# szbonaldo/FedMLP

Hardware: AMD Instinct MI355X
Metric: images/sec/client (ICH 224x224 bs=128) at 1/2/4/8 GPUs; mAP vs ref (higher is better)
Workload: dtype f32; 1 GPU; FedMLP stage1 step, Resnet18, ICH-shaped synthetic 3x224x224, C=5, bs=128, one client per GPU, FedAvg all-reduce every 40 steps + once at end; parallelism=clients1, rccl_ranks=1, stream_mode=default: frozen teacher + weight gradients on the engine's side stream, arithmetic=fp32 operands+sums; products as 6 exact bf16 partials on the bf16 matrix pipe

## Files before the change

### fedmlp_amd/_lib.py

```python
import ctypes as C
import os

_HERE = os.path.dirname(os.path.abspath(__file__))
LIB_PATH = os.environ.get("FEDMLP_HIP_LIB") or os.path.join(_HERE, "libfedmlp_hip.so")

FM_MAX_CLASSES = 32
FM_MAX_GROUPS = 8
FM_COMM_ID_BYTES = 128


class FmConfig(C.Structure):
    _fields_ = [("model", C.c_int32), ("n_classes", C.c_int32), ("in_h", C.c_int32),
                ("in_w", C.c_int32), ("max_images", C.c_int32), ("reserved", C.c_int32 * 3),
                ("stream", C.c_void_p)]


class FmAdam(C.Structure):
    _fields_ = [("lr", C.c_float), ("beta1", C.c_float), ("beta2", C.c_float),
                ("eps", C.c_float), ("weight_decay", C.c_float)]


class FmSgd(C.Structure):
    _fields_ = [("lr", C.c_float), ("momentum", C.c_float), ("dampening", C.c_float),
                ("weight_decay", C.c_float), ("nesterov", C.c_int32)]
# ... 86 lines not shown
    "fm_comm_preflight": (C.c_int, []),
    "fm_comm_unique_id": (C.c_int, [C.POINTER(C.c_uint8)]),
    "fm_comm_init": (C.c_int, [_P, C.POINTER(C.c_uint8), _I32, _I32]),
    "fm_comm_destroy": (C.c_int, [_P]),
    "fm_comm_size": (C.c_int, [_P]),
    "fm_fedavg_allreduce": (C.c_int, [_P, C.c_float]),
    "fm_fedavg_tao": (C.c_int, [_P, C.POINTER(C.c_double), C.c_double, _F, C.POINTER(C.c_double)]),
    "fm_fedavg_proto": (C.c_int, [_P, _P, C.c_double, _F, _P]),
    "fm_profile_ops": (C.c_int, [_P, _I32, C.c_char_p, _I32]),
    "fm_debug_num_convs": (C.c_int, [_P]),
    "fm_debug_conv_info": (C.c_int, [_P, _I32, C.POINTER(_I32)]),
    "fm_debug_conv": (C.c_int, [_P, _I32, _I32, _P, _P, _P, _I32, _I32, _P]),
    "fm_debug_conv_fwd": (C.c_int, [_P, _I32, _P, _P, _I32, _I32, _P, _P, _P, _I32, _P, _P, _P, _P]),
    "fm_debug_block_dgrad": (C.c_int, [_P, _I32, _P, _P, _P, _I32]),
    "fm_debug_conv_planes": (C.c_int, [_P, _I32, _P, _I32, _P, _P, _P, _P, _I32, _P, _P]),
    "fm_debug_conv_arm": (C.c_int, [_P, _I32, _I32, _I32]),
    "fm_debug_pw": (C.c_int, [_P, _I32, _I32, _P, _P, _P, _I32, _I32, _P, _P, _P, _P]),
    "fm_debug_pw_fwd": (C.c_int, [_P, _I32, _P, _P, _I32, _I32, _P, _P, _P, _I32, _P, _P, _P, _P]),
    "fm_debug_proj_bwd": (C.c_int, [_P, _I32, _I32, _P, _P, _P, _P, _P, _I32, _I32, _P, _P]),
    "fm_debug_exp_bwd": (C.c_int, [_P, _I32, _P, _P, _P, _P, _P, _I32, _I32, _P, _P]),
    "fm_debug_get_grads": (C.c_int, [_P, _P]),
    "fm_debug_optim_arena": (C.c_int, [_P, _I32, C.POINTER(_P), C.POINTER(_I64)]),
    "fm_debug_entry_spans": (C.c_int, [_P, _P, _I32]),
    "fm_debug_activation": (C.c_int, [_P, _I32, _I32, _I32, _P, C.POINTER(_I32)]),
    "fm_debug_stem_masks": (C.c_int, [_P, _I32, _I32, _P, _P]),
    "fm_debug_lose_part": (C.c_int, [_I32]),
    "fm_debug_lane_delay": (C.c_int, [_P, _I32, _I64, _I32]),
    "fm_debug_lane_points": (C.c_int, [_P, C.POINTER(_I64), _I32]),
    "fm_debug_drop_wait": (C.c_int, [_P, _I32, _I32]),
    "fm_debug_ew": (C.c_int, [_P, _I32, C.POINTER(_P), C.POINTER(_I32), _F]),
# ... 59 lines not shown
```

### fedmlp_amd/csrc/common.h

```cpp
#pragma once
#include <hip/hip_runtime.h>
#include <stdint.h>

#include <stdlib.h>

typedef float f32x4 __attribute__((ext_vector_type(4)));

#ifndef FM_F32_FAST_SWISH
#define FM_F32_FAST_SWISH 1
#endif
#ifdef __HIPCC__
__device__ __forceinline__ float fm_swish_f32(float v)
{
#if FM_F32_FAST_SWISH
    return v * __builtin_amdgcn_rcpf(1.f + __expf(-v));
#else
    return v / (1.f + expf(-v));
#endif
}
#endif


#ifndef FM_MFMA_SPLIT_DEFAULT
#define FM_MFMA_SPLIT_DEFAULT 6
// ... 151 lines not shown
    int Ho, Wo, Hi, Wi, Ci, stride, pad, ksz;
    long long npix, xpix;
    int pix_per_split;
    int tilesM, tilesN, nblk_n;
    int sp;
    int nimg, Qtot, q_per_split, splits, xcd_remap;
    unsigned magW, magH;
};
struct StemRowsParams {
    const unsigned short* Xp;
    const unsigned short* Wst;
    float* Y;
    const float* scale;
    const float* shift;
    float* stats;
    int imgs, imgs_per_group, Hp, Wp, Ho, Wo, relu, sp;
    long long plane_bytes;
};
bool stem_rows_takes(int k, int stride, int cout, int hout, int wout, long long plane_bytes);
int stem_rows_stats_tiles(int imgs_per_group, int hout);
void launch_stem_rows(StemRowsParams p, hipStream_t s);
void k_stem_weight_planes(const float* w, unsigned short* dst, int Kw, hipStream_t s);
int launch_pwgrad(PwgradParams p, size_t slab_floats, hipStream_t s);
bool pwgrad_ring_takes(const PwgradParams& p);
int launch_pwgrad_ring(PwgradParams p, size_t slab_floats, hipStream_t s);
bool pwgrad_takes(int M, int Ci, int ksz, long long npix, long long xpix, int Wi, int pad);
void launch_igemm(IgemmParams p, int groups, hipStream_t s);
void launch_pconv(IgemmParams p, int groups, hipStream_t s);
bool pconv_takes(int M, int Ci, long long xp_pix, int Wi);
bool pconv_uses_ts(const IgemmParams& p);
// ... 20 lines not shown
```

### fedmlp_amd/csrc/engine.hip

```cpp
#include <math.h>
#include <stdio.h>
#include <string.h>

#include <algorithm>
#include <string>
#include <unordered_map>
#include <vector>

#include "../../include/fedmlp_hip.h"
#include "../../include/fedmlp_hip_debug.h"
#include "../../include/fedmlp_hip_rofl.h"
#include "../../include/fedmlp_hip_drift.h"
#include "comm.h"
#include "common.h"
#include "kernels.h"
#include "pwconv.h"

static thread_local std::string g_err;
const char* fm_last_error(void) { return g_err.c_str(); }
const char* fm_version(void) { return "fedmlp_hip 0.2 (gfx950)"; }

#define HIPCHK(x)                                                                              \
    do {                                                                                       \
        hipError_t e_ = (x);                                                                   \
// ... 84 lines not shown
struct In { const float* f = nullptr; const unsigned short* p = nullptr; };
struct Out {
    float* f = nullptr; unsigned short* p = nullptr;
    operator In() const { return {f, p}; }
};
inline Out kept(Out t) { return t.p ? Out{nullptr, t.p} : t; }

struct BlockActs {
    Out z1, out;
    float* ds_y = nullptr;
};
struct MBActs { float *a_e = nullptr, *y_d = nullptr, *a_s = nullptr, *out = nullptr, *sq = nullptr, *rpre = nullptr, *gate = nullptr; };
struct Acts {
    float* stem_y = nullptr;
    Out p0;
    float* a0 = nullptr;
    std::vector<BlockActs> blk;
    std::vector<MBActs> mb;
    float *T_mid = nullptr, *se_pool = nullptr;
};

enum class BnMode { Batch, BatchNoUpdate, Frozen };
struct Bwd {
    bool frozen = false;
    const float* dfeat = nullptr;
    float* dx[2] = {nullptr, nullptr};
    bool step = true;
    const int32_t* train = nullptr;
};

// ... 570 lines not shown
    const Conv& chd = e->convs[e->c_head];
    z.t_mid = std::max(z.t_mid, B * chd.hout * chd.wout * chd.cout_p);
    return z;
}

int alloc_acts(fm_engine* e, Acts& a, bool second)
{
    const size_t B = e->maxB;
    const Conv& c0 = e->convs[0];
    if (e->model == 0) {
        const size_t pooled = B * (c0.hout / 2) * (c0.wout / 2) * 64;
        a.stem_y = c0.y;
        if (second) DALLOC(a.stem_y, B * c0.hout * c0.wout * c0.cout_p);
        DALLOC(a.p0.f, pooled);
        if (e->planes) PALLOC(a.p0.p, pooled);
        a.blk.resize(e->blocks.size());
        for (size_t i = 0; i < e->blocks.size(); ++i) {
            const Block& blk = e->blocks[i];
            BlockActs& ba = a.blk[i];
            const Conv& c = e->convs[blk.c1];
            const size_t n = B * c.hout * c.wout * c.cout;
            DALLOC(ba.z1.f, n); DALLOC(ba.out.f, n);
            if (blk.ds >= 0) {
                ba.ds_y = e->convs[blk.ds].y;
                if (second) DALLOC(ba.ds_y, n);
            }
            if (e->planes) { PALLOC(ba.z1.p, n); PALLOC(ba.out.p, n); }
        }
        return FM_OK;
    }
// ... 216 lines not shown
            if (e->op_names[i] == lab) { id = (int)i; break; }
        if (id < 0) { id = (int)e->op_names.size(); e->op_names.push_back(lab); e->op_ms.push_back(0); e->op_n.push_back(0); }
        a = get_ev(e); b = get_ev(e);
        on = a && b && hipEventRecord(a, st) == hipSuccess;
    }
    ~OpScope()
    {
        if (on && hipEventRecord(b, st) == hipSuccess) e->opevs.push_back({a, b, id});
    }
};
#define OP(lane, name) OpScope os_(e, lane, name)
#define LP(lane) lane_point(e, &(lane) == &e->side)

struct Prologue { const float *psc = nullptr, *psh = nullptr, *gate = nullptr; };
enum { ACT_NONE = 0, ACT_RELU = 1, ACT_SWISH = 2 };
struct Epilogue { const float *scale = nullptr, *shift = nullptr; In res; int act = ACT_NONE; };
struct FwdOps { float* stats = nullptr; Prologue pro; Epilogue epi; };

const unsigned short* scratch_planes(fm_engine* e, Lane& L, const float* x, long long npix, int C)
{
    if ((size_t)npix * C * 3 > e->xp_scratch_elems) { soft(e, hipErrorInvalidValue); return nullptr; }
    static const bool reuse = getenv("FM_DEBUG_REUSE_PLANES") && atoi(getenv("FM_DEBUG_REUSE_PLANES")) != 0;
    if (reuse && e->xp_scratch_src == x && e->xp_scratch_npix == npix) return e->xp_scratch;
    k_split_planes(x, e->xp_scratch, npix, C, L.st);
    e->xp_scratch_src = x; e->xp_scratch_npix = npix;
    return e->xp_scratch;
}
bool conv_uses_pconv(const fm_engine* e, const Conv& c, int imgs)
{
    return e->planes && c.pl_off >= 0 && pconv_takes(c.cout_p, c.cin_p, (long long)imgs * c.hin * c.win, c.win);
}
// ... 114 lines not shown
    default: return tiles(igemm_tile_n(c.cout_p, c.cin == 3));
    }
}

void conv_fwd(fm_engine* e, Lane& L, int ci, const Weights& W, In x, Out y, int imgs, int groups, const FwdOps& o = {})
{
    Conv& c = e->convs[ci];
    const Epilogue& ep = o.epi;
    const Prologue& pro = o.pro;
    float* const stats = o.stats;
    const Arm arm = fwd_arm(e, c, imgs);
    const int tiles_n = stats_tiles_for(arm, c, imgs / groups, groups, pro.gate != nullptr);
    if (stats) { e->stats_conv = ci; e->stats_tiles_n = tiles_n; }
    const int fam = prof_family(arm, c.cout_p);
    const double flops = 2.0 * c.macs_per_img * imgs;
    switch (arm) {
    case Arm::StemRows: {
        StemRowsParams q{};
        q.Xp = e->x3p + (size_t)e->in_img0 * c.Hp * c.Wp * 4; q.Wst = W.wst; q.Y = y.f;
        q.scale = ep.scale; q.shift = ep.shift; q.stats = stats; q.relu = ep.act;
        q.imgs = imgs; q.imgs_per_group = imgs / groups; q.Hp = c.Hp; q.Wp = c.Wp; q.Ho = c.hout; q.Wo = c.wout;
        q.sp = e->products; q.plane_bytes = e->x3p_plane_elems * 2;
        ProfScope ps(e, L, fam, flops);
        launch_stem_rows(q, L.st);
        return;
    }
    case Arm::PwConv: {
        const bool stem16 = c.cin == 3;
        PwParams q{};
        q.zeros = e->zeros;
        q.W = W.wb + c.wb_off;
        q.X = reinterpret_cast<const bf16*>(stem16 ? e->stem_col : x.f); q.Y = reinterpret_cast<bf16*>(y.f);
        if (stem16) q.X += (size_t)e->in_img0 * c.hout * c.wout * c.Kw;
// ... 257 lines not shown
{
    const Out y{e->convs[ci].y};
    const FwdOps o{.stats = e->ws_stats, .pro = pro};
    if (op) {
        { OP(L, op); conv_fwd(e, L, ci, W, x, y, groups * B, groups, o); }
        { OP(L, "bn_fwd_finalize"); bn_fwd_finalize(e, L, ci, groups, B, mode); }
    } else {
        LP(L); conv_fwd(e, L, ci, W, x, y, groups * B, groups, o);
        LP(L); bn_fwd_finalize(e, L, ci, groups, B, mode);
    }
}
void conv_fwd_eval(fm_engine* e, Lane& L, int ci, const Weights& W, In x, Out y, int imgs, int act, In res = {}, const Prologue& pro = {})
{
    const int ch = e->bns[e->convs[ci].bn].ch_off;
    conv_fwd(e, L, ci, W, x, y, imgs, 1, {.pro = pro, .epi = {W.ev_scale + ch, W.ev_shift + ch, res, act}});
}

void bn_bwd_finalize(fm_engine* e, Lane& L, const Bn& b, int groups, int partials, int count, bool frozen)
{
    const BnSlots s = bn_slots(e, b);
    k_bn_bwd_finalize(e->ws_part, groups, partials, b.C, count, s.gamma, b.mean, b.istd, e->ca, e->cb, e->cc, s.dgamma, s.dbeta, L.st, frozen);
}
enum class Mask { None, Z, ZPlane, OwnOutput };
void bn_bwd(fm_engine* e, Lane& L, int bi, const float* dz, Out dy, int groups, int imgs_per_group, bool frozen, Mask mask = Mask::None,
            In z = {}, float* dyh_out = nullptr)
{
    const Conv& c = e->convs[bi];
    Bn& b = e->bns[bi];
    const int pix = imgs_per_group * c.hout * c.wout;
    const char* fy = getenv("FM_BN_MASK_FROM_Y");
// ... 115 lines not shown
            apply(blk.c2, out, idt);
        }
        cur = out;
    }
    const Conv& cl = e->convs[e->blocks.back().c2];
    LP(L); k_avgpool(cur.f, DT_F32, e->feat, imgs, cl.hout * cl.wout, 512, L.st);
    LP(L); k_fc_fwd(e->feat, S + e->off_fcw, S + e->off_fcb, e->logits, imgs, 512, e->C, L.st);
    if (mode != BnMode::Frozen) net_changed(e, e->student, Moved::Stats);
}

void forward_eval(fm_engine* e, Lane& L, Weights& W, Acts& A, int imgs, float* feat, float* logits)
{
    const float* S = W.state;
    LP(L); ensure_eval_affine(e, L, W);
    Conv& c0 = e->convs[0];
    LP(L); conv_fwd_eval(e, L, 0, W, {e->x4}, {A.stem_y}, imgs, ACT_RELU);
    LP(L);
    if (A.p0.p) k_stem_pool_planes(A.stem_y, nullptr, nullptr, A.p0.f, nullptr, A.p0.p, 1, imgs, c0.hout, c0.wout, 64, L.st);
    else k_stem_pool(A.stem_y, nullptr, nullptr, A.p0.f, nullptr, 1, imgs, c0.hout, c0.wout, 64, L.st);
    In cur = A.p0;
    for (size_t bi = 0; bi < e->blocks.size(); ++bi) {
        const Block& blk = e->blocks[bi];
        BlockActs& a = A.blk[bi];
        const bool last = bi + 1 == e->blocks.size();
        LP(L); conv_fwd_eval(e, L, blk.c1, W, cur, kept(a.z1), imgs, ACT_RELU);
        In idt = cur.f ? In{cur.f} : cur;
        if (blk.ds >= 0) {
            LP(L); conv_fwd_eval(e, L, blk.ds, W, cur, {a.ds_y}, imgs, ACT_NONE);
            idt = {a.ds_y};
        }
        const Out out = last ? Out{a.out.f} : kept(a.out);
        LP(L); conv_fwd_eval(e, L, blk.c2, W, kept(a.z1), out, imgs, ACT_RELU, idt);
        cur = out;
    }
// ... 2393 lines not shown
    ARGCHK(e->model == 0 && !e->precision && e->planes, "fm_debug_conv_planes: a planes-mode precision-0 ResNet-18 engine");
    ARGCHK(scale_dev && shift_dev, "the eval epilogue needs scale and shift");
    ARGCHK(imgs >= 1 && imgs <= e->maxB, "imgs");
    ARGCHK(relu == 0 || relu == 1, "relu");
    ARGCHK(!(res_dev && resp_dev), "one residual form: fp32 or planes");
    ARGCHK(out_dev || outp_dev, "an output: fp32, planes or both");
    Conv& c = e->convs[conv];
    ARGCHK(c.cin != 3 && conv_uses_pconv(e, c, imgs), "a convolution the planes kernel runs (not the stem)");
    ensure_packed(e);
    conv_fwd(e, e->main, conv, e->student, {.p = xp_dev}, {out_dev, outp_dev}, imgs, 1, {.epi = {scale_dev, shift_dev, {res_dev, resp_dev}, relu}});
    HIPCHK(hipStreamSynchronize(e->main.st));
    STEP_DONE(e);
    return FM_OK;
}

int fm_debug_conv_arm(fm_engine* e, int32_t op, int32_t conv, int32_t imgs)
{
    ARGCHK(e && conv >= 0 && conv < (int)e->convs.size(), "conv index");
    ARGCHK(!e->precision, "fm_debug_conv_arm: a precision-0 engine");
    ARGCHK(imgs >= 1 && imgs <= e->maxB && op >= 0 && op <= 2, "imgs / op");
    const Conv& c = e->convs[conv];
    if (op == 1 && c.cin == 3) return FM_ARM_STEM_DGRAD;
    ARGCHK(op != 1 || c.ncls > 0, "dgrad unavailable for this conv");
    switch (op == 0 ? fwd_arm(e, c, imgs) : (op == 1 ? dgrad_arm(e, c, imgs) : wgrad_arm(e, c, imgs))) {
    case Arm::StemRows: return FM_ARM_STEM_ROWS;
    case Arm::PconvTs: return FM_ARM_PCONV_TS;
    case Arm::PconvTap: return FM_ARM_PCONV_TAP;
    case Arm::Igemm: return FM_ARM_IGEMM;
    case Arm::IgemmStem: return FM_ARM_IGEMM_STEM;
    case Arm::Pwgrad: return FM_ARM_PWGRAD;
// ... 336 lines not shown
```

### fedmlp_amd/csrc/kernels.h

```cpp
#pragma once
#include <hip/hip_runtime.h>
#include <stdint.h>

#include "common.h"

#define FM_MAXC 32

struct ClassVec { float v[FM_MAXC]; };
struct TapList { int t[9]; int n; };

void k_nchw_to_nhwc4(const float* x, float* y, int imgs, int H, int W, hipStream_t s);
void k_stem_im2col(const float* x, void* col, int imgs, int H, int W, int Ho, int Wo, int k, int stride, int pad_t, int pad_l,
                   hipStream_t s);
void k_oihw_to_ohwi(const float* src, float* dst, int O, int I, int H, int W, int Wpad, int Ipad, hipStream_t s, int Ostride = 0);
void k_ohwi_to_oihw(const float* src, float* dst, int O, int I, int H, int W, int Wpad, int Ipad, hipStream_t s, int Ostride = 0);
void k_stem3_mask_grad(float* g, int O, hipStream_t s);
void k_frame_nhwc3(const float* x, float* y, int imgs, int H, int W, int Hp, int Wp, int top, int left, int src_nhwc3,
                   hipStream_t s, unsigned short* yp = nullptr, long long yp_plane_elems = 0);
void k_pack_dgrad(const float* w, float* out, int Co, int T, int Ci, TapList taps, hipStream_t s);
struct PackJob { long long w_off; float* out; int Co, T, Ci, ntaps; int taps[9]; int blk0; };
void k_pack_dgrad_all(const float* state, const PackJob* jobs, int njobs, int nblocks, hipStream_t s);
int pack_job_blocks(int Co, int Ci, int ntaps);
struct SplitJob { long long src_off; const float* src; long long dst_off; int M, ntaps, cib, blk0; };
inline int split_job_blocks(int M, int ntaps, int cib) { return (int)(((long long)M * ntaps * cib * 4 + 255) / 256); }
void k_split_weights(const float* src_base, unsigned short* dst_base, const SplitJob* jobs, int njobs, int nblocks, hipStream_t s);
void k_split_weights_bm(const float* src_base, unsigned short* dst_base, const SplitJob* jobs, int njobs, int nblocks, hipStream_t s);
void k_split_planes(const float* x, unsigned short* dst, long long npix, int C, hipStream_t s);
void k_planes_to_f32(const unsigned short* src, float* x, long long npix, int C, hipStream_t s);
void k_bn_apply_planes(const float* y, const float* scale, const float* shift, const float* res, const float* y2, const float* scale2,
                       const float* shift2, float* out, unsigned short* outp, int groups, int pix_per_group, int C, int relu,
                       hipStream_t s, const unsigned short* resp = nullptr);
void k_stem_pool_planes(const float* y, const float* scale, const float* shift, float* pooled, uint8_t* idx, unsigned short* pooledp,
                        int groups, int imgs_per_group, int H, int W, int C, hipStream_t s);
void k_bn_bwd_apply_planes(const float* dz, const float* z, const float* y, const float* ca, const float* cb, const float* cc, float* dy,
                           unsigned short* dyp, float* dyh_out, int groups, int pix_per_group, int C, hipStream_t s,
                           const float* mask_scale = nullptr, const float* mask_shift = nullptr, const unsigned short* zh = nullptr);
void k_scale(float* x, float w, int64_t n, hipStream_t s);
#define FM_FOLD_MAX 16
struct FoldArgs { const float* s[FM_FOLD_MAX]; float n[FM_FOLD_MAX]; };
void k_fedavg_fold(const FoldArgs& a, int K, float tot, float* out, int64_t n, hipStream_t s);
void k_axpby(float* y, const float* x, float a, float b, int64_t n, hipStream_t s);
#define FM_DIST_CHUNK 8192
struct DistEntry { long long off; int len, row, dense, Ipad, I, Wpad, W, chunk0, nchunks, all_real; };
struct DistChunk { int entry, start; };
void k_state_dist(const FoldArgs& a, int K, const float* ref, const DistEntry* ent, int n_entries, const DistChunk* chunks,
                  int n_chunks, int64_t NS, double* part, float* norms, hipStream_t s);

#define FM_METRICS_ROWS 64
// ... 180 lines not shown
```

### fedmlp_amd/csrc/planes_ew.hip

```cpp
#include "common.h"
#include "kernels.h"
#include "split3.h"

static inline int pe_cdiv(int64_t a, int64_t b) { return (int)((a + b - 1) / b); }

#if __HIP_DEVICE_COMPILE__
__device__ __forceinline__ size_t pe_off(int c, int64_t pix, int64_t P)
{
    return (((size_t)(c >> 5) * 3) * P + pix) * 64 + ((c & 15) >> 2) * 16 + ((c >> 4) & 1) * 8;
}
__device__ __forceinline__ void pe_store_planes(unsigned short* planes, int64_t P, int c, int64_t pix, f32x4 v, bool active)
{
    f32x4 up;
#pragma unroll
    for (int k = 0; k < 4; ++k) up[k] = __shfl_down(v[k], 4);
    if (active && (c & 16) == 0) {
        sp_u32x4 H, M, L;
        split3(v, up, H, M, L);
        unsigned char* d = reinterpret_cast<unsigned char*>(planes) + (((size_t)(c >> 5) * 3) * P + pix) * 64 + ((c & 15) >> 2) * 16;
        *reinterpret_cast<sp_u32x4*>(d) = H;
        *reinterpret_cast<sp_u32x4*>(d + (size_t)P * 64) = M;
        *reinterpret_cast<sp_u32x4*>(d + (size_t)P * 128) = L;
    }
}
__device__ __forceinline__ f32x4 pe_load_planes(const unsigned short* planes, int64_t P, int c, int64_t pix)
{
    const unsigned char* s = reinterpret_cast<const unsigned char*>(planes) + pe_off(c, pix, P);
    const uint2 H = *reinterpret_cast<const uint2*>(s);
    const uint2 M = *reinterpret_cast<const uint2*>(s + (size_t)P * 64);
    const uint2 L = *reinterpret_cast<const uint2*>(s + (size_t)P * 128);
    f32x4 v;
    v[0] = (__builtin_bit_cast(float, H.x << 16) + __builtin_bit_cast(float, M.x << 16)) + __builtin_bit_cast(float, L.x << 16);
    v[1] = (__builtin_bit_cast(float, H.x & 0xffff0000u) + __builtin_bit_cast(float, M.x & 0xffff0000u)) + __builtin_bit_cast(float, L.x & 0xffff0000u);
    v[2] = (__builtin_bit_cast(float, H.y << 16) + __builtin_bit_cast(float, M.y << 16)) + __builtin_bit_cast(float, L.y << 16);
    v[3] = (__builtin_bit_cast(float, H.y & 0xffff0000u) + __builtin_bit_cast(float, M.y & 0xffff0000u)) + __builtin_bit_cast(float, L.y & 0xffff0000u);
    return v;
}
__device__ __forceinline__ f32x4 pe_mask_h(f32x4 d, const unsigned short* zh, int64_t P, int c, int64_t pix)
// ... 102 lines not shown
        if (idx)
            *reinterpret_cast<uchar4*>(idx + o) = make_uchar4((unsigned char)code[0], (unsigned char)code[1], (unsigned char)code[2],
                                                              (unsigned char)code[3]);
    }
    pe_store_planes(pooledp, (int64_t)gridDim.y * ppg, c, (int64_t)grp * ppg + pixg, best, active);
#endif
}
void k_stem_pool_planes(const float* y, const float* scale, const float* shift, float* pooled, uint8_t* idx, unsigned short* pooledp,
                        int groups, int imgs_per_group, int H, int W, int C, hipStream_t s)
{
    const int64_t n = (int64_t)imgs_per_group * (H / 2) * (W / 2) * (C / 4);
    hipLaunchKernelGGL(stem_pool_planes_kernel, dim3(pe_cdiv(n, 256), groups), dim3(256), 0, s, y, scale, shift, pooled, idx, pooledp,
                       imgs_per_group, H, W, C);
}

__global__ __launch_bounds__(256) void bn_bwd_apply_planes_kernel(const float* __restrict__ dz, const float* __restrict__ z,
                                                                  const float* __restrict__ y, const float* __restrict__ ca,
                                                                  const float* __restrict__ cb_, const float* __restrict__ cc, float* dy,
                                                                  unsigned short* __restrict__ dyp, float* dyh_out, int pix_per_group,
                                                                  int C, const float* __restrict__ msc, const float* __restrict__ msh,
                                                                  const unsigned short* __restrict__ zh)
{
#if __HIP_DEVICE_COMPILE__
    const int grp = blockIdx.y;
    const int Q = C >> 2;
    const int64_t n4 = (int64_t)pix_per_group * Q;
    const int64_t P = (int64_t)gridDim.y * pix_per_group;
    const int64_t i = (int64_t)blockIdx.x * 256 + threadIdx.x;
    const bool active = i < n4;
    const int64_t ii = active ? i : 0;
// ... 33 lines not shown
```

### fedmlp_amd/csrc/split3.h

```cpp
#pragma once
#include "common.h"

#if defined(__HIPCC__)
typedef unsigned int sp_u32x4 __attribute__((ext_vector_type(4)));
typedef float sp_f32x2 __attribute__((ext_vector_type(2)));
typedef __bf16 sp_bf16x2 __attribute__((ext_vector_type(2)));

__device__ __forceinline__ float sp_sub(float a, float b)
{
#ifdef FM_SPLIT_PK
    return a - b;
#else
    float r;
    asm("v_sub_f32_e32 %0, %1, %2" : "=v"(r) : "v"(a), "v"(b));
    return r;
#endif
}
__device__ __forceinline__ void split3_pair(const sp_f32x2 e, unsigned& H, unsigned& M, unsigned& L)
{
    const unsigned hw = __builtin_bit_cast(unsigned, __builtin_convertvector(e, sp_bf16x2));
    const sp_f32x2 r = {sp_sub(e.x, __builtin_bit_cast(float, hw << 16)), sp_sub(e.y, __builtin_bit_cast(float, hw & 0xffff0000u))};
    const unsigned mw = __builtin_bit_cast(unsigned, __builtin_convertvector(r, sp_bf16x2));
    const sp_f32x2 l = {sp_sub(r.x, __builtin_bit_cast(float, mw << 16)), sp_sub(r.y, __builtin_bit_cast(float, mw & 0xffff0000u))};
    H = hw;
// ... 20 lines not shown
                                            const sp_u32x4 bm, const sp_u32x4 bl, f32x4 v)
{
    if constexpr (SP == 9) {
        v = mfma_bf16(al, bl, v);
        v = mfma_bf16(al, bm, v);
        v = mfma_bf16(am, bl, v);
    }
    v = mfma_bf16(al, bh, v);
    v = mfma_bf16(ah, bl, v);
    v = mfma_bf16(am, bm, v);
    v = mfma_bf16(am, bh, v);
    v = mfma_bf16(ah, bm, v);
    v = mfma_bf16(ah, bh, v);
    return v;
}
#endif
```

### fedmlp_amd/csrc/stem_rows.hip

```cpp
#include <stdlib.h>

#include <algorithm>
#include <type_traits>

#include "common.h"
#include "kernels.h"
#include "split3.h"

#if __HIP_DEVICE_COMPILE__
template <int IMM> __device__ __forceinline__ sp_u32x4 sr_lds_read128(unsigned addr)
{
    sp_u32x4 v;
    asm volatile("ds_read_b128 %0, %1 offset:%2" : "=v"(v) : "v"(addr), "n"(IMM));
    return v;
}
template <int CTRL> __device__ __forceinline__ float sr_dpp(float v)
{
    return __builtin_bit_cast(float, __builtin_amdgcn_update_dpp(0, __builtin_bit_cast(int, v), CTRL, 0xF, 0xF, false));
}
#endif

namespace {
constexpr int SR_WBYTES = 7 * 3 * 64 * 64;
constexpr int SR_PLANE = 24 * 1024;
constexpr int SR_LDS = SR_WBYTES + 3 * SR_PLANE + 4 * 64 * 2 * 4;
}

template <int SP>
__global__ __launch_bounds__(512, 2) void stem_rows_kernel(const StemRowsParams p)
{
#if __HIP_DEVICE_COMPILE__
    constexpr int FR = 2, FC = 7;
    typedef __attribute__((address_space(3))) void lds_void;
    extern __shared__ __attribute__((aligned(16))) unsigned char smem[];
// ... 78 lines not shown
        f32x4 scv[FR], shv[FR];
        if (p.scale) {
#pragma unroll
            for (int r = 0; r < FR; ++r) {
                scv[r] = *reinterpret_cast<const f32x4*>(p.scale + mbase + 16 * r);
                shv[r] = *reinterpret_cast<const f32x4*>(p.shift + mbase + 16 * r);
            }
        }
#pragma unroll
        for (int c = 0; c < FC; ++c) {
            float* o = p.Y + (((size_t)img * Ho + oh) * Wo + 16 * c + li) * 64;
#pragma unroll
            for (int r = 0; r < FR; ++r) {
                const int m = mbase + 16 * r;
                f32x4 v = a[r][c];
                if (p.scale) v = v * scv[r] + shv[r];
                if (p.relu == 1) {
#pragma unroll
                    for (int q = 0; q < 4; ++q) v[q] = fmaxf(v[q], 0.f);
                }
                *reinterpret_cast<f32x4*>(o + m) = v;
            }
        }
    };
    if ((int)blockIdx.x < ntiles) load_rows(blockIdx.x);
    for (int tile = blockIdx.x; tile < ntiles; tile += gridDim.x) {
        asm volatile("s_waitcnt vmcnt(0)" ::: "memory");
        __builtin_amdgcn_s_barrier();
        asm volatile("" ::: "memory");

        f32x4 acc[FR][FC];
#pragma unroll
        for (int r = 0; r < FR; ++r)
#pragma unroll
            for (int c = 0; c < FC; ++c) acc[r][c] = f32x4{0.f, 0.f, 0.f, 0.f};
        sp_u32x4 A0[FR][3], A1[FR][3], Bb[3][3];
#define SR_READA(KH, DST)                                                                        \
    {                                                                                            \
// ... 33 lines not shown
        SR_READA(0, A0);
        SR_READB(Bf, 0, Bb[0]);
        SR_READB(Bf, 1, Bb[1]);
        SR_LGKM0();
#define SR_G(N) column(std::integral_constant<int, N>{});
#define SR_G7(N) SR_G(N) SR_G(N + 1) SR_G(N + 2) SR_G(N + 3) SR_G(N + 4) SR_G(N + 5) SR_G(N + 6)
        SR_G7(0) SR_G7(7) SR_G7(14) SR_G7(21) SR_G7(28) SR_G7(35) SR_G7(42)
#undef SR_G7
#undef SR_G
#undef SR_MFMA
#undef SR_READB
#undef SR_READA
        asm volatile("s_waitcnt lgkmcnt(0)" ::: "memory");
        __builtin_amdgcn_s_barrier();
        asm volatile("" ::: "memory");
        if (tile + (int)gridDim.x < ntiles) load_rows(tile + gridDim.x);

        epilogue(acc, tile);
    }
#undef SR_LGKM0
#endif
}

__global__ __launch_bounds__(256) void stem_weight_planes_kernel(const float* __restrict__ w, unsigned short* __restrict__ dst, int Kw)
{
#if __HIP_DEVICE_COMPILE__
    const int idx = blockIdx.x * 256 + threadIdx.x;
    if (idx >= 7 * 64 * 4) return;
    const int g = idx & 3, m = (idx >> 2) & 63, kh = idx >> 8;
    float v[8];
#pragma unroll
    for (int e = 0; e < 8; ++e) {
        const int kw = 2 * g + (e >> 2), c = e & 3;
// ... 35 lines not shown
```

### fedmlp_amd/engine.py

```python
import ctypes as C

import numpy as np
import torch

from . import _lib, spec

MODEL_IDS = {"Resnet18": 0, "Efficient_b0": 1}
PRECISION_IDS = {"fp32": 0, "bf16": 1}
PRODUCT_FORMS = {None: 0, 6: 3, 0: 1, 9: 2}


def _ptr(t):
    if t is None:
        return None
    assert t.is_cuda and t.is_contiguous() and t.dtype in (torch.float32, torch.int32, torch.bfloat16), \
        (t.device, t.dtype, t.is_contiguous())
    return C.c_void_p(t.data_ptr())


def _cargs(args):
    return [_ptr(a) if torch.is_tensor(a) else a for a in args]


class RoflHeads:
# ... 752 lines not shown

    def debug_conv_fwd(self, conv, x, out, imgs, groups=1, scale=None, shift=None, res=None, act=0, psc=None, psh=None,
                       gate=None, stats=None):
        self._enqueue()
        _lib.check(self.lib.fm_debug_conv_fwd(self.h, conv, _ptr(x), _ptr(out), imgs, groups, _ptr(scale), _ptr(shift),
                                              _ptr(res), int(act), _ptr(psc), _ptr(psh), _ptr(gate), _ptr(stats)))

    def debug_conv_planes(self, conv, xp, imgs, scale, shift, res=None, resp=None, relu=0, out=None, outp=None):
        def words(t):
            assert t is None or (t.is_cuda and t.is_contiguous() and t.dtype == torch.int16), "planes are int16 device tensors"
            return None if t is None else C.c_void_p(t.data_ptr())
        self._enqueue()
        _lib.check(self.lib.fm_debug_conv_planes(self.h, conv, words(xp), imgs, _ptr(scale), _ptr(shift), _ptr(res), words(resp),
                                                 int(relu), _ptr(out), words(outp)))

    CONV_ARMS = ("igemm", "igemm_stem", "stem_rows", "pconv_ts", "pconv_tap", "pwgrad", "pwgrad_ring", "wgrad_generic",
                 "wgrad_skinny", "stem_dgrad")

    def debug_conv_arm(self, op, conv, imgs):
        rc = self.lib.fm_debug_conv_arm(self.h, op, conv, imgs)
        if rc < 0:
            _lib.check(rc)
        return self.CONV_ARMS[rc]

    def debug_block_dgrad(self, block, dy1, dyd, dx, imgs):
        self._enqueue()
        _lib.check(self.lib.fm_debug_block_dgrad(self.h, block, _ptr(dy1), _ptr(dyd), _ptr(dx), imgs))

    EW_OPS = ("split_planes", "planes_to_f32", "bn_finalize", "bn_finalize_frozen", "bn_eval_affine", "bn_apply",
              "bn_apply_planes", "stem_pool", "stem_pool_planes", "stem_pool_bwd", "stem_pool_bn_reduce", "stem_pool_bn_apply",
# ... 93 lines not shown
```

### include/fedmlp_hip_debug.h

```cpp
#ifndef FEDMLP_HIP_DEBUG_H
#define FEDMLP_HIP_DEBUG_H

#include "fedmlp_hip.h"

#ifdef __cplusplus
extern "C" {
#endif

int fm_debug_conv_info(fm_engine* e, int32_t conv, int32_t* info16);
int fm_debug_num_convs(fm_engine* e);
int fm_debug_conv(fm_engine* e, int32_t op, int32_t conv, const float* x_dev, const float* dy_dev,
                  float* out_dev, int32_t imgs, int32_t groups, float* stats_dev);

int fm_debug_conv_fwd(fm_engine* e, int32_t conv, const float* x_dev, float* out_dev, int32_t imgs, int32_t groups,
                      const float* scale_dev, const float* shift_dev, const float* res_dev, int32_t act, const float* psc_dev,
                      const float* psh_dev, const float* gate_dev, float* stats_dev);

int fm_debug_conv_planes(fm_engine* e, int32_t conv, const uint16_t* xp_dev, int32_t imgs, const float* scale_dev,
                         const float* shift_dev, const float* res_dev, const uint16_t* resp_dev, int32_t relu, float* out_dev,
                         uint16_t* outp_dev);

enum { FM_ARM_IGEMM = 0, FM_ARM_IGEMM_STEM, FM_ARM_STEM_ROWS, FM_ARM_PCONV_TS, FM_ARM_PCONV_TAP, FM_ARM_PWGRAD, FM_ARM_PWGRAD_RING,
       FM_ARM_WGRAD_GENERIC, FM_ARM_WGRAD_SKINNY, FM_ARM_STEM_DGRAD };
int fm_debug_conv_arm(fm_engine* e, int32_t op, int32_t conv, int32_t imgs);

int fm_debug_block_dgrad(fm_engine* e, int32_t block, const float* dy1_dev, const float* dyd_dev, float* dx_dev, int32_t imgs);

int fm_debug_pw(fm_engine* e, int32_t op, int32_t conv, const void* x_dev, const void* dy_dev, void* out_dev,
                int32_t imgs, int32_t groups, const float* psc_dev, const float* psh_dev, const float* gate_dev,
                float* stats_dev);

int fm_debug_pw_fwd(fm_engine* e, int32_t conv, const void* x_dev, void* out_dev, int32_t imgs, int32_t groups,
                    const float* scale_dev, const float* shift_dev, const void* res_dev, int32_t act, const float* psc_dev,
                    const float* psh_dev, const float* gate_dev, float* stats_dev);

// ... 54 lines not shown
```

Before: 6187 images/sec.

## Fuse stem max-pool into stem_rows conv epilogue for the frozen teacher eval path

On the eval (teacher) forward, the stem convolution on the stem_rows arm now applies BN affine and ReLU and then max-pools 3x3/2 directly in its epilogue. Horizontal maxima are taken with DPP lane moves and staged rows go through shared memory; the row at each tile boundary is written to a halo buffer. A small finish kernel then merges that halo row and writes the pooled output plus its bf16 split planes. This avoids writing and re-reading the full dense stem activation map, at the cost of an extra barrier-heavy epilogue, an extra launch and a halo allocation.

New measurement: 6168 images/sec. Within noise of the previous version (-0.3%).

```diff
diff --git a/fedmlp_amd/_lib.py b/fedmlp_amd/_lib.py
--- a/fedmlp_amd/_lib.py
+++ b/fedmlp_amd/_lib.py
@@ -124,6 +124,7 @@
     "fm_debug_conv_fwd": (C.c_int, [_P, _I32, _P, _P, _I32, _I32, _P, _P, _P, _I32, _P, _P, _P, _P]),
     "fm_debug_block_dgrad": (C.c_int, [_P, _I32, _P, _P, _P, _I32]),
     "fm_debug_conv_planes": (C.c_int, [_P, _I32, _P, _I32, _P, _P, _P, _P, _I32, _P, _P]),
+    "fm_debug_stem_eval_pool": (C.c_int, [_P, _P, _I32, _I32, _P, _P, _I32, _P, _P, _P, _P]),
     "fm_debug_conv_arm": (C.c_int, [_P, _I32, _I32, _I32]),
     "fm_debug_pw": (C.c_int, [_P, _I32, _I32, _P, _P, _P, _I32, _I32, _P, _P, _P, _P]),
     "fm_debug_pw_fwd": (C.c_int, [_P, _I32, _P, _P, _I32, _I32, _P, _P, _P, _I32, _P, _P, _P, _P]),
diff --git a/fedmlp_amd/csrc/common.h b/fedmlp_amd/csrc/common.h
--- a/fedmlp_amd/csrc/common.h
+++ b/fedmlp_amd/csrc/common.h
@@ -189,6 +189,9 @@
     const float* scale;
     const float* shift;
     float* stats;
+    float* pool_f;
+    unsigned short* pool_p;
+    float* pool_halo;
     int imgs, imgs_per_group, Hp, Wp, Ho, Wo, relu, sp;
     long long plane_bytes;
 };
diff --git a/fedmlp_amd/csrc/engine.hip b/fedmlp_amd/csrc/engine.hip
--- a/fedmlp_amd/csrc/engine.hip
+++ b/fedmlp_amd/csrc/engine.hip
@@ -122,6 +122,7 @@
 struct Acts {
     float* stem_y = nullptr;
     Out p0;
+    float* stem_halo = nullptr;
     float* a0 = nullptr;
     std::vector<BlockActs> blk;
     std::vector<MBActs> mb;
@@ -722,6 +723,7 @@
         if (second) DALLOC(a.stem_y, B * c0.hout * c0.wout * c0.cout_p);
         DALLOC(a.p0.f, pooled);
         if (e->planes) PALLOC(a.p0.p, pooled);
+        if (e->stem_rows) DALLOC(a.stem_halo, pooled / 2);
         a.blk.resize(e->blocks.size());
         for (size_t i = 0; i < e->blocks.size(); ++i) {
             const Block& blk = e->blocks[i];
@@ -968,7 +970,7 @@
 
 struct Prologue { const float *psc = nullptr, *psh = nullptr, *gate = nullptr; };
 enum { ACT_NONE = 0, ACT_RELU = 1, ACT_SWISH = 2 };
-struct Epilogue { const float *scale = nullptr, *shift = nullptr; In res; int act = ACT_NONE; };
+struct Epilogue { const float *scale = nullptr, *shift = nullptr; In res; int act = ACT_NONE; Out pool; float* pool_halo = nullptr; };
 struct FwdOps { float* stats = nullptr; Prologue pro; Epilogue epi; };
 
 const unsigned short* scratch_planes(fm_engine* e, Lane& L, const float* x, long long npix, int C)
@@ -1113,9 +1115,15 @@
     if (stats) { e->stats_conv = ci; e->stats_tiles_n = tiles_n; }
     const int fam = prof_family(arm, c.cout_p);
     const double flops = 2.0 * c.macs_per_img * imgs;
+    if ((ep.pool.f || ep.pool.p || ep.pool_halo) &&
+        (arm != Arm::StemRows || !ep.pool.f || !ep.pool_halo || !ep.scale || ep.act != ACT_RELU || stats || groups != 1)) {
+        soft(e, hipErrorInvalidValue);
+        return;
+    }
     switch (arm) {
     case Arm::StemRows: {
         StemRowsParams q{};
+        q.pool_f = ep.pool.f; q.pool_p = ep.pool.p; q.pool_halo = ep.pool_halo;
         q.Xp = e->x3p + (size_t)e->in_img0 * c.Hp * c.Wp * 4; q.Wst = W.wst; q.Y = y.f;
         q.scale = ep.scale; q.shift = ep.shift; q.stats = stats; q.relu = ep.act;
         q.imgs = imgs; q.imgs_per_group = imgs / groups; q.Hp = c.Hp; q.Wp = c.Wp; q.Ho = c.hout; q.Wo = c.wout;
@@ -1403,6 +1411,12 @@
 {
     const int ch = e->bns[e->convs[ci].bn].ch_off;
     conv_fwd(e, L, ci, W, x, y, imgs, 1, {.pro = pro, .epi = {W.ev_scale + ch, W.ev_shift + ch, res, act}});
+}
+void conv_fwd_eval_pooled(fm_engine* e, Lane& L, int ci, const Weights& W, Out pool, float* pool_halo, int imgs)
+{
+    const int ch = e->bns[e->convs[ci].bn].ch_off;
+    conv_fwd(e, L, ci, W, {e->x4}, {}, imgs, 1,
+             {.epi = {.scale = W.ev_scale + ch, .shift = W.ev_shift + ch, .act = ACT_RELU, .pool = pool, .pool_halo = pool_halo}});
 }
 
 void bn_bwd_finalize(fm_engine* e, Lane& L, const Bn& b, int groups, int partials, int count, bool frozen)
@@ -1548,10 +1562,15 @@
     const float* S = W.state;
     LP(L); ensure_eval_affine(e, L, W);
     Conv& c0 = e->convs[0];
-    LP(L); conv_fwd_eval(e, L, 0, W, {e->x4}, {A.stem_y}, imgs, ACT_RELU);
-    LP(L);
-    if (A.p0.p) k_stem_pool_planes(A.stem_y, nullptr, nullptr, A.p0.f, nullptr, A.p0.p, 1, imgs, c0.hout, c0.wout, 64, L.st);
-    else k_stem_pool(A.stem_y, nullptr, nullptr, A.p0.f, nullptr, 1, imgs, c0.hout, c0.wout, 64, L.st);
+    if (fwd_arm(e, c0, imgs) == Arm::StemRows) {
+        LP(L); conv_fwd_eval_pooled(e, L, 0, W, A.p0, A.stem_halo, imgs);
+        LP(L); k_stem_pool_finish_planes(A.p0.f, A.stem_halo, A.p0.f, A.p0.p, imgs, c0.hout / 2, c0.wout / 2, 64, L.st);
+    } else {
+        LP(L); conv_fwd_eval(e, L, 0, W, {e->x4}, {A.stem_y}, imgs, ACT_RELU);
+        LP(L);
+        if (A.p0.p) k_stem_pool_planes(A.stem_y, nullptr, nullptr, A.p0.f, nullptr, A.p0.p, 1, imgs, c0.hout, c0.wout, 64, L.st);
+        else k_stem_pool(A.stem_y, nullptr, nullptr, A.p0.f, nullptr, 1, imgs, c0.hout, c0.wout, 64, L.st);
+    }
     In cur = A.p0;
     for (size_t bi = 0; bi < e->blocks.size(); ++bi) {
         const Block& blk = e->blocks[bi];
@@ -3975,6 +3994,36 @@
     return FM_OK;
 }
 
+int fm_debug_stem_eval_pool(fm_engine* e, const float* x_dev, int32_t imgs, int32_t in_img0, const float* scale_dev,
+                            const float* shift_dev, int32_t fused, float* dense_dev, float* pooled_dev, uint16_t* planes_dev,
+                            float* halo_dev)
+{
+    ARGCHK(e && x_dev && scale_dev && shift_dev && pooled_dev && planes_dev, "null tensor");
+    ARGCHK(e->model == 0 && !e->precision, "fm_debug_stem_eval_pool: a precision-0 ResNet-18 engine");
+    ARGCHK(imgs >= 1 && in_img0 >= 0 && in_img0 + imgs <= e->maxB, "imgs / in_img0");
+    ARGCHK(fused == 0 || fused == 1, "fused");
+    ARGCHK(fused ? halo_dev != nullptr : dense_dev != nullptr, "the dense map (fused 0) or the halo rows (fused 1)");
+    Conv& c = e->convs[0];
+    ARGCHK(fwd_arm(e, c, imgs) == Arm::StemRows, "the stem of this handle does not run on stem_rows");
+    Lane& L = e->main;
+    k_frame_nhwc3(x_dev, e->x3, in_img0 + imgs, c.hin, c.win, c.Hp, c.Wp, 3, 3, 1, L.st, e->x3p, e->x3p_plane_elems);
+    ensure_packed(e);
+    const int img0 = e->in_img0;
+    e->in_img0 = in_img0;
+    if (fused) {
+        conv_fwd(e, L, 0, e->student, {}, {}, imgs, 1,
+                 {.epi = {.scale = scale_dev, .shift = shift_dev, .act = ACT_RELU, .pool = {pooled_dev, planes_dev}, .pool_halo = halo_dev}});
+        k_stem_pool_finish_planes(pooled_dev, halo_dev, pooled_dev, planes_dev, imgs, c.hout / 2, c.wout / 2, 64, L.st);
+    } else {
+        conv_fwd(e, L, 0, e->student, {}, {dense_dev}, imgs, 1, {.epi = {.scale = scale_dev, .shift = shift_dev, .act = ACT_RELU}});
+        k_stem_pool_planes(dense_dev, nullptr, nullptr, pooled_dev, nullptr, planes_dev, 1, imgs, c.hout, c.wout, 64, L.st);
+    }
+    e->in_img0 = img0;
+    HIPCHK(hipStreamSynchronize(L.st));
+    STEP_DONE(e);
+    return FM_OK;
+}
+
 int fm_debug_conv_arm(fm_engine* e, int32_t op, int32_t conv, int32_t imgs)
 {
     ARGCHK(e && conv >= 0 && conv < (int)e->convs.size(), "conv index");
diff --git a/fedmlp_amd/csrc/kernels.h b/fedmlp_amd/csrc/kernels.h
--- a/fedmlp_amd/csrc/kernels.h
+++ b/fedmlp_amd/csrc/kernels.h
@@ -32,6 +32,8 @@
                        hipStream_t s, const unsigned short* resp = nullptr);
 void k_stem_pool_planes(const float* y, const float* scale, const float* shift, float* pooled, uint8_t* idx, unsigned short* pooledp,
                         int groups, int imgs_per_group, int H, int W, int C, hipStream_t s);
+void k_stem_pool_finish_planes(const float* partial, const float* halo, float* pooled, unsigned short* pooledp, int imgs, int Hp, int Wp,
+                               int C, hipStream_t s);
 void k_bn_bwd_apply_planes(const float* dz, const float* z, const float* y, const float* ca, const float* cb, const float* cc, float* dy,
                            unsigned short* dyp, float* dyh_out, int groups, int pix_per_group, int C, hipStream_t s,
                            const float* mask_scale = nullptr, const float* mask_shift = nullptr, const unsigned short* zh = nullptr);
diff --git a/fedmlp_amd/csrc/planes_ew.hip b/fedmlp_amd/csrc/planes_ew.hip
--- a/fedmlp_amd/csrc/planes_ew.hip
+++ b/fedmlp_amd/csrc/planes_ew.hip
@@ -8,20 +8,6 @@
 __device__ __forceinline__ size_t pe_off(int c, int64_t pix, int64_t P)
 {
     return (((size_t)(c >> 5) * 3) * P + pix) * 64 + ((c & 15) >> 2) * 16 + ((c >> 4) & 1) * 8;
-}
-__device__ __forceinline__ void pe_store_planes(unsigned short* planes, int64_t P, int c, int64_t pix, f32x4 v, bool active)
-{
-    f32x4 up;
-#pragma unroll
-    for (int k = 0; k < 4; ++k) up[k] = __shfl_down(v[k], 4);
-    if (active && (c & 16) == 0) {
-        sp_u32x4 H, M, L;
-        split3(v, up, H, M, L);
-        unsigned char* d = reinterpret_cast<unsigned char*>(planes) + (((size_t)(c >> 5) * 3) * P + pix) * 64 + ((c & 15) >> 2) * 16;
-        *reinterpret_cast<sp_u32x4*>(d) = H;
-        *reinterpret_cast<sp_u32x4*>(d + (size_t)P * 64) = M;
-        *reinterpret_cast<sp_u32x4*>(d + (size_t)P * 128) = L;
-    }
 }
 __device__ __forceinline__ f32x4 pe_load_planes(const unsigned short* planes, int64_t P, int c, int64_t pix)
 {
@@ -154,6 +140,43 @@
                        imgs_per_group, H, W, C);
 }
 
+__global__ __launch_bounds__(256) void stem_pool_finish_planes_kernel(const float* partial, const float* __restrict__ halo,
+                                                                      float* pooled, unsigned short* __restrict__ pooledp, int imgs,
+                                                                      int Hp, int Wp, int C)
+{
+#if __HIP_DEVICE_COMPILE__
+    const int Q = C >> 2, T = Hp >> 1;
+    const int64_t n = (int64_t)imgs * T * Wp * Q;
+    const int64_t i0 = (int64_t)blockIdx.x * 256 + threadIdx.x;
+    const bool active = i0 < n;
+    const int64_t i = active ? i0 : 0;
+    const int c = (int)(i % Q) * 4;
+    int64_t r = i / Q;
+    const int ow = (int)(r % Wp); r /= Wp;
+    const int t = (int)(r % T);
+    const int img = (int)(r / T);
+    const int64_t pix = ((int64_t)img * Hp + 2 * t) * Wp + ow;
+    const f32x4 a = ld4(partial + (size_t)pix * C + c);
+    const f32x4 h = ld4(halo + ((size_t)((int64_t)img * T + (t ? t - 1 : 0)) * Wp + ow) * C + c);
+    f32x4 best = {-INFINITY, -INFINITY, -INFINITY, -INFINITY};
+#pragma unroll
+    for (int k = 0; k < 4; ++k) {
+        const float u = t ? h[k] : -INFINITY;
+        if (u > best[k]) best[k] = u;
+        if (a[k] > best[k]) best[k] = a[k];
+    }
+    if (active && pooled) st4(pooled + (size_t)pix * C + c, best);
+    if (pooledp) pe_store_planes(pooledp, (int64_t)imgs * Hp * Wp, c, pix, best, active);
+#endif
+}
+void k_stem_pool_finish_planes(const float* partial, const float* halo, float* pooled, unsigned short* pooledp, int imgs, int Hp, int Wp,
+                               int C, hipStream_t s)
+{
+    const int64_t n = (int64_t)imgs * (Hp / 2) * Wp * (C / 4);
+    hipLaunchKernelGGL(stem_pool_finish_planes_kernel, dim3(pe_cdiv(n, 256)), dim3(256), 0, s, partial, halo, pooled, pooledp, imgs, Hp,
+                       Wp, C);
+}
+
 __global__ __launch_bounds__(256) void bn_bwd_apply_planes_kernel(const float* __restrict__ dz, const float* __restrict__ z,
                                                                   const float* __restrict__ y, const float* __restrict__ ca,
                                                                   const float* __restrict__ cb_, const float* __restrict__ cc, float* dy,
diff --git a/fedmlp_amd/csrc/split3.h b/fedmlp_amd/csrc/split3.h
--- a/fedmlp_amd/csrc/split3.h
+++ b/fedmlp_amd/csrc/split3.h
@@ -58,4 +58,18 @@
     v = mfma_bf16(ah, bh, v);
     return v;
 }
+__device__ __forceinline__ void pe_store_planes(unsigned short* planes, int64_t P, int c, int64_t pix, f32x4 v, bool active)
+{
+    f32x4 up;
+#pragma unroll
+    for (int k = 0; k < 4; ++k) up[k] = __shfl_down(v[k], 4);
+    if (active && (c & 16) == 0) {
+        sp_u32x4 H, M, L;
+        split3(v, up, H, M, L);
+        unsigned char* d = reinterpret_cast<unsigned char*>(planes) + (((size_t)(c >> 5) * 3) * P + pix) * 64 + ((c & 15) >> 2) * 16;
+        *reinterpret_cast<sp_u32x4*>(d) = H;
+        *reinterpret_cast<sp_u32x4*>(d + (size_t)P * 64) = M;
+        *reinterpret_cast<sp_u32x4*>(d + (size_t)P * 128) = L;
+    }
+}
 #endif
diff --git a/fedmlp_amd/csrc/stem_rows.hip b/fedmlp_amd/csrc/stem_rows.hip
--- a/fedmlp_amd/csrc/stem_rows.hip
+++ b/fedmlp_amd/csrc/stem_rows.hip
@@ -18,6 +18,18 @@
 {
     return __builtin_bit_cast(float, __builtin_amdgcn_update_dpp(0, __builtin_bit_cast(int, v), CTRL, 0xF, 0xF, false));
 }
+template <int CTRL> __device__ __forceinline__ float sr_dpp_old(float old, float v)
+{
+    return __builtin_bit_cast(float, __builtin_amdgcn_update_dpp(__builtin_bit_cast(int, old), __builtin_bit_cast(int, v), CTRL, 0xF, 0xF, false));
+}
+__device__ __forceinline__ f32x4 sr_affine(f32x4 v, f32x4 sc, f32x4 sh) { return v * sc + sh; }
+__device__ __forceinline__ f32x4 sr_relu(f32x4 v)
+{
+#pragma unroll
+    for (int q = 0; q < 4; ++q) v[q] = fmaxf(v[q], 0.f);
+    return v;
+}
+__device__ __forceinline__ float sr_pick(float best, float u) { return u > best ? u : best; }
 #endif
 
 namespace {
@@ -126,14 +138,74 @@
             for (int r = 0; r < FR; ++r) {
                 const int m = mbase + 16 * r;
                 f32x4 v = a[r][c];
-                if (p.scale) v = v * scv[r] + shv[r];
-                if (p.relu == 1) {
-#pragma unroll
-                    for (int q = 0; q < 4; ++q) v[q] = fmaxf(v[q], 0.f);
-                }
+                if (p.scale) v = sr_affine(v, scv[r], shv[r]);
+                if (p.relu == 1) v = sr_relu(v);
                 *reinterpret_cast<f32x4*>(o + m) = v;
             }
         }
+    };
+    constexpr int PW = 56, PROW = PW * 256;
+    static_assert(4 * PROW <= 3 * SR_PLANE, "the staged rows fit the input-row region");
+    auto epilogue_pool = [&](const f32x4 (&a)[FR][FC], int tile) {
+        const int img = tile / tiles_per_img, t4 = tile - img * tiles_per_img;
+        const int mbase = 32 * wm + 4 * lg;
+        f32x4 z[FR][FC];
+#pragma unroll
+        for (int r = 0; r < FR; ++r) {
+            const f32x4 sc = *reinterpret_cast<const f32x4*>(p.scale + mbase + 16 * r);
+            const f32x4 sh = *reinterpret_cast<const f32x4*>(p.shift + mbase + 16 * r);
+#pragma unroll
+            for (int c = 0; c < FC; ++c) z[r][c] = sr_relu(sr_affine(a[r][c], sc, sh));
+        }
+        unsigned char* const stage = smem + SR_WBYTES;
+#pragma unroll
+        for (int r = 0; r < FR; ++r) {
+#pragma unroll
+            for (int c = 0; c < FC; ++c) {
+                f32x4 h;
+#pragma unroll
+                for (int q = 0; q < 4; ++q) {
+                    const float ctr = z[r][c][q];
+                    const float edge = c ? sr_dpp<0x121>(z[r][c ? c - 1 : 0][q]) : -INFINITY;
+                    const float lft = sr_dpp_old<0x111>(edge, ctr);
+                    const float rgt = sr_dpp<0xF5>(ctr);
+                    h[q] = sr_pick(sr_pick(sr_pick(-INFINITY, lft), ctr), rgt);
+                }
+                if ((li & 1) == 0) {
+                    const int ow = 8 * c + (li >> 1);
+                    const int chunk = (8 * wm + 4 * r + lg) ^ ((ow & 3) << 2);
+                    *reinterpret_cast<f32x4*>(stage + wn * PROW + ow * 256 + chunk * 16) = h;
+                }
+            }
+        }
+        asm volatile("s_waitcnt lgkmcnt(0)" ::: "memory");
+        __builtin_amdgcn_s_barrier();
+        asm volatile("" ::: "memory");
+        const int Hq = Ho >> 1;
+        for (int g = wave; g < 3 * 14; g += 8) {
+            const int kind = g / 14, gg = g - 14 * kind;
+            const int ow = 4 * gg + (lane >> 4), cq = lane & 15;
+            const unsigned char* const src = stage + ow * 256 + ((cq ^ ((ow & 3) << 2)) << 4);
+            auto row = [&](int rr) { return *reinterpret_cast<const f32x4*>(src + rr * PROW); };
+            f32x4 best;
+            if (kind == 2) {
+                best = row(3);
+                *reinterpret_cast<f32x4*>(p.pool_halo + (((size_t)img * tiles_per_img + t4) * PW + ow) * 64 + 4 * cq) = best;
+                continue;
+            }
+            const f32x4 u0 = row(kind), u1 = row(kind + 1), u2 = row(kind ? 3 : 1);
+#pragma unroll
+            for (int q = 0; q < 4; ++q) {
+                best[q] = sr_pick(sr_pick(-INFINITY, u0[q]), u1[q]);
+                if (kind) best[q] = sr_pick(best[q], u2[q]);
+            }
+            const size_t pix = ((size_t)img * Hq + 2 * t4 + kind) * PW + ow;
+            *reinterpret_cast<f32x4*>(p.pool_f + pix * 64 + 4 * cq) = best;
+            if (kind && p.pool_p) pe_store_planes(p.pool_p, (int64_t)p.imgs * Hq * PW, 4 * cq, (int64_t)pix, best, true);
+        }
+        asm volatile("s_waitcnt lgkmcnt(0)" ::: "memory");
+        __builtin_amdgcn_s_barrier();
+        asm volatile("" ::: "memory");
     };
     if ((int)blockIdx.x < ntiles) load_rows(blockIdx.x);
     for (int tile = blockIdx.x; tile < ntiles; tile += gridDim.x) {
@@ -197,9 +269,13 @@
         asm volatile("s_waitcnt lgkmcnt(0)" ::: "memory");
         __builtin_amdgcn_s_barrier();
         asm volatile("" ::: "memory");
-        if (tile + (int)gridDim.x < ntiles) load_rows(tile + gridDim.x);
-
-        epilogue(acc, tile);
+        if (p.pool_f) {
+            epilogue_pool(acc, tile);
+            if (tile + (int)gridDim.x < ntiles) load_rows(tile + gridDim.x);
+        } else {
+            if (tile + (int)gridDim.x < ntiles) load_rows(tile + gridDim.x);
+            epilogue(acc, tile);
+        }
     }
 #undef SR_LGKM0
 #endif
diff --git a/fedmlp_amd/engine.py b/fedmlp_amd/engine.py
--- a/fedmlp_amd/engine.py
+++ b/fedmlp_amd/engine.py
@@ -790,6 +790,12 @@
         _lib.check(self.lib.fm_debug_conv_planes(self.h, conv, words(xp), imgs, _ptr(scale), _ptr(shift), _ptr(res), words(resp),
                                                  int(relu), _ptr(out), words(outp)))
 
+    def debug_stem_eval_pool(self, x, imgs, scale, shift, fused, pooled, planes, dense=None, halo=None, in_img0=0):
+        assert planes.is_cuda and planes.is_contiguous() and planes.dtype == torch.int16, "planes are int16 device tensors"
+        self._enqueue()
+        _lib.check(self.lib.fm_debug_stem_eval_pool(self.h, _ptr(x), imgs, in_img0, _ptr(scale), _ptr(shift), int(bool(fused)),
+                                                    _ptr(dense), _ptr(pooled), C.c_void_p(planes.data_ptr()), _ptr(halo)))
+
     CONV_ARMS = ("igemm", "igemm_stem", "stem_rows", "pconv_ts", "pconv_tap", "pwgrad", "pwgrad_ring", "wgrad_generic",
                  "wgrad_skinny", "stem_dgrad")
 
diff --git a/include/fedmlp_hip_debug.h b/include/fedmlp_hip_debug.h
--- a/include/fedmlp_hip_debug.h
+++ b/include/fedmlp_hip_debug.h
@@ -19,6 +19,10 @@
 int fm_debug_conv_planes(fm_engine* e, int32_t conv, const uint16_t* xp_dev, int32_t imgs, const float* scale_dev,
                          const float* shift_dev, const float* res_dev, const uint16_t* resp_dev, int32_t relu, float* out_dev,
                          uint16_t* outp_dev);
+
+int fm_debug_stem_eval_pool(fm_engine* e, const float* x_dev, int32_t imgs, int32_t in_img0, const float* scale_dev,
+                            const float* shift_dev, int32_t fused, float* dense_dev, float* pooled_dev, uint16_t* planes_dev,
+                            float* halo_dev);
 
 enum { FM_ARM_IGEMM = 0, FM_ARM_IGEMM_STEM, FM_ARM_STEM_ROWS, FM_ARM_PCONV_TS, FM_ARM_PCONV_TAP, FM_ARM_PWGRAD, FM_ARM_PWGRAD_RING,
        FM_ARM_WGRAD_GENERIC, FM_ARM_WGRAD_SKINNY, FM_ARM_STEM_DGRAD };
```
